# cerbos/cerbos

Measured on AMD Instinct MI355X. Metric: CheckResources decisions/sec at batch=1M; p50 per-decision us, higher is better.
Workload: dtype u32 ids + f64 attributes (CEL int64/uint64/double)

## Files before the change

### __graft_entry__.py

```python
from __future__ import annotations

import glob
import os
import subprocess
import sys

ROOT = os.path.dirname(os.path.abspath(__file__))
if ROOT not in sys.path:
    sys.path.insert(0, ROOT)

CSRC = os.path.join(ROOT, "cerbos_amd", "csrc")
LIB = os.path.join(ROOT, "cerbos_amd", "libcerbos_hip.so")
SOURCES = ["cbh_engine.hip", "cbh_host_env.h", "cbh_host_resident.h", "cbh_host_cross.h", "cbh_host_wire.h", "cbh_host_oneshot.h", "cbh_kernels.h", "cbh_check_wave.h", "cbh_check_flat.h", "cbh_check_walk2.h", "cbh_interp.h", "cbh_vm.h", "cbh_blob.h", "cbh_image.h",
           "cbh_wire.h", "cbh_wire_host.h", "cbh_wire_req.h", "cbh_cross.h"]


def _stale(target, deps):
    if not os.path.exists(target):
        return True
    t = os.path.getmtime(target)
    return any(os.path.getmtime(d) > t for d in deps)


def build() -> None:
    deps = [os.path.join(CSRC, s) for s in SOURCES] + [os.path.join(ROOT, "include", "cerbos_hip.h")]
    if _stale(LIB, deps):
        hipcc = os.environ.get("HIPCC", "/opt/rocm/bin/hipcc")
        cmd = [hipcc, "--offload-arch=gfx950", "-O3", "-std=c++17", "-shared", "-fPIC",
# ... 89 lines not shown
```

### cerbos_amd/csrc/cbh_check_flat.h

```cpp
#pragma once
#include "cbh_check_wave.h"

#define CBH_FLAT_MAX_DEPTH 16
#if defined(CBH_FLAT_WAVES_OVERRIDE)
#define CBH_FLAT_WAVES CBH_FLAT_WAVES_OVERRIDE
#elif !defined(CBH_HOSTSIM)
#define CBH_FLAT_WAVES 4u
#else
#define CBH_FLAT_WAVES 1u
#endif
#define CBH_FLAT_THREADS (CBH_FLAT_WAVES * CBH_BLOCK)

__device__ __forceinline__ u64 wave_or64(u64 v, u32 wave, u32 lane) {
  __shared__ unsigned long long acc[CBH_FLAT_WAVES];
#ifndef CBH_HOSTSIM
  if (lane == 0) __hip_atomic_store(&acc[wave], 0ull, __ATOMIC_RELAXED, __HIP_MEMORY_SCOPE_WORKGROUP);
  (void)wave_ballot(true);
  if (v) (void)__hip_atomic_fetch_or(&acc[wave], (unsigned long long)v, __ATOMIC_RELAXED, __HIP_MEMORY_SCOPE_WORKGROUP);
  (void)wave_ballot(true);
  const u64 r = __hip_atomic_load(&acc[wave], __ATOMIC_RELAXED, __HIP_MEMORY_SCOPE_WORKGROUP);
#else
  if (lane == 0) acc[wave] = 0;
  (void)wave_ballot(true);
  if (v) atomicOr(&acc[wave], (unsigned long long)v);
// ... 1169 lines not shown
__global__ __launch_bounds__(256) void cbh_unpack_results_kernel(PkUnpackArgs a) {
  const u32 i = blockIdx.x * 256u + threadIdx.x;
  if (i >= a.n) return;
  const u32 w = a.policy[i];
  a.effect[i] = (u8)cbh_pk_effect(w); a.status[i] = (u8)cbh_pk_status(w);
  a.policy[i] = cbh_pk_policy(w, a.bits); a.scope[i] = cbh_pk_scope(w, a.bits);
}
struct CompactArgs {
  const CBH_G u32* req_u32; const CBH_G u32* roles; const CBH_G u32* tuple_action; const CBH_G u64* col_val;
  const CBH_G u8* action_class; const CBH_G u8* role_class;
  const CBH_G u8* col_tag; CBH_G u32* ctag;
  CBH_G u32* creq; CBH_G u32* cval; CBH_G u32* info;
  u32 n_requests, n_cached, K, narrow;
  const CBH_G u32* scope_parent; const CBH_G u32* scope_flags; u32 n_scopes;
};
__global__ __launch_bounds__(256) void cbh_compact_scan_kernel(CompactArgs a) {
  const u32 r = blockIdx.x * 256u + threadIdx.x;
  if (r >= a.n_requests) return;
  const size_t NR = a.n_requests;
  u32 m = 0;
  for (u32 k = 0; k < a.n_cached; ++k) m |= (u32)(a.col_val[k * NR + r] >> 32) ? 1u << k : 0u;
#define RQ(f) a.req_u32[(size_t)(f) * NR + r]
  if ((RQ(CBH_RQ_KIND) | RQ(CBH_RQ_R_VERSION) | (RQ(CBH_RQ_R_SCOPE) & ~CBH_SCOPE_EXACT)) >> 16) m |= CBH_CI_MISFIT;
  if (RQ(CBH_RQ_ROLE_CNT) > 4u || RQ(CBH_RQ_ACT_CNT) > 4u) m |= CBH_CI_MISFIT;
  if (RQ(CBH_RQ_ACT_OFF) != 4u * r || RQ(CBH_RQ_ACT_CNT) != 4u) m |= CBH_CI_ACT4;
#undef RQ
#ifdef CBH_HOSTSIM
  a.info[0] |= m;
#else
  if (m & ~__hip_atomic_load(a.info, __ATOMIC_RELAXED, __HIP_MEMORY_SCOPE_AGENT)) atomicOr((unsigned int*)a.info, m);
// ... 11 lines not shown
  u32 ac[4], rc[4];
  for (u32 k = 0; k < 4; ++k) {
    const u32 aid = a.tuple_action[k < act_cnt ? act_off + k : 0u], rid = a.roles[k < role_cnt ? role_off + k : 0u];
    const u32 ca = a.K ? a.action_class[aid < a.K ? aid : kmax] : 31u, cr = a.K ? a.role_class[rid < a.K ? rid : kmax] : 31u;
    ac[k] = (k < act_cnt && aid < a.K && ca < 31u) ? ca : 31u;
    rc[k] = (k < role_cnt && rid < a.K && cr < 31u) ? cr : 31u;
  }
  const u32 si = r_scope & ~CBH_SCOPE_EXACT;
  u32 first = CBH_NONE;
  bool strict = false;
  if (si < a.n_scopes) {
    strict = (r_scope & CBH_SCOPE_EXACT) != 0 && (a.scope_flags[si] & FLAG_RES) != 0;
    first = si;
    while (first != CBH_NONE && !(a.scope_flags[first] & FLAG_RES)) first = a.scope_parent[first];
  }
  CBH_G u32* rec = a.creq + 4u * (size_t)r;
  rec[0] = pid; rec[1] = cbh_creq_w1(kind, r_ver);
  rec[2] = cbh_creq_w2(first, role_cnt, act_cnt, rc[2], rc[3]);
  rec[3] = cbh_creq_w3(first, strict, ac[0], ac[1], ac[2], ac[3], rc[0], rc[1]);
  u32 plane = 0;
  for (u32 k = 0; k < a.n_cached; ++k)
    if ((a.narrow >> k) & 1u) { a.cval[plane * NR + r] = (u32)a.col_val[k * NR + r]; ++plane; }
  for (u32 g = 0; 4u * g < a.n_cached; ++g) {
    u32 w = 0;
    for (u32 j = 0; j < 4u && 4u * g + j < a.n_cached; ++j) w |= (u32)a.col_tag[(4u * g + j) * NR + r] << (8u * j);
    a.ctag[g * NR + r] = w;
  }
}
static inline cbh_check_kernel_fn cbh_flat_compact_variant(cbh_check_kernel_fn fn) {
  return fn == cbh_check_flat_kernel ? cbh_check_flat_kernel_c
// ... 29 lines not shown
  const int m = cbh_flat_cross_mode(fn);
  return m == 0 ? cbh_check_flat_kernel_x : m == 1 ? cbh_check_flat_kernel_staged_x : m == 2 ? cbh_check_flat_kernel_masks_x : m == 3 ? cbh_check_flat_kernel_dr_x : nullptr;
}
static inline const char* cbh_flat_cross_name(cbh_check_kernel_fn fn) {
  const int m = cbh_flat_cross_mode(fn);
  return m == 0 ? "cbh_check_flat_kernel_x" : m == 1 ? "cbh_check_flat_kernel_staged_x" : m == 2 ? "cbh_check_flat_kernel_masks_x" : m == 3 ? "cbh_check_flat_kernel_dr_x" : "";
}
#define CBH_FLAT_STAGE_MIN 32u
static inline bool cbh_flat_use_masks(const void* segs, u32 max_bucket) {
  static const char* e = getenv("CBH_FLAT_MASKS");
  static const bool force_staged = getenv("CBH_FORCE_STAGED") != nullptr;
  if ((e && *e == '0') || force_staged) return false;
  return segs != nullptr && ((e && *e == '1') || max_bucket > CBH_FLAT_STAGE_MIN);
}

static inline size_t cbh_flat_chain_bytes(u32 table_max_depth, u32 table_scopes) {
  return (size_t)(table_max_depth < CBH_FLAT_MAX_DEPTH ? table_max_depth : CBH_FLAT_MAX_DEPTH) * CBH_BLOCK * (table_scopes <= 256u ? 1 : 4);
}
static inline size_t cbh_flat_class_bytes(u32 table_strings) {
  return table_strings <= CBH_FLAT_LDS_STRINGS ? (((size_t)2 * table_strings + 15) & ~(size_t)15) : 0;
}
static inline size_t cbh_flat_mask_bytes(u32 threads) { return (size_t)(threads / CBH_BLOCK) * CBH_SEG_LDS_BYTES; }
static inline bool cbh_is_mask_kernel(cbh_check_kernel_fn fn) {
  return fn == cbh_check_flat_kernel_masks || fn == cbh_check_flat_kernel_any_masks || fn == cbh_check_flat_trail_kernel_masks || fn == cbh_check_flat_trail_kernel_any_masks;
}
static inline cbh_check_kernel_fn cbh_flat_trail_variant(cbh_check_kernel_fn fn) {
  return (fn == cbh_check_flat_kernel || fn == cbh_check_flat_kernel_dr) ? cbh_check_flat_trail_kernel : fn == cbh_check_flat_kernel_any ? cbh_check_flat_trail_kernel_any
       : fn == cbh_check_flat_kernel_staged ? cbh_check_flat_trail_kernel_staged : fn == cbh_check_flat_kernel_any_staged ? cbh_check_flat_trail_kernel_any_staged
       : fn == cbh_check_flat_kernel_masks ? cbh_check_flat_trail_kernel_masks : fn == cbh_check_flat_kernel_any_masks ? cbh_check_flat_trail_kernel_any_masks : fn;
}
static inline bool cbh_is_flat_trail_kernel(cbh_check_kernel_fn fn) {
  return fn == cbh_check_flat_trail_kernel || fn == cbh_check_flat_trail_kernel_any || fn == cbh_check_flat_trail_kernel_staged ||
         fn == cbh_check_flat_trail_kernel_any_staged || fn == cbh_check_flat_trail_kernel_masks || fn == cbh_check_flat_trail_kernel_any_masks;
}
// ... 18 lines not shown
```

### cerbos_amd/csrc/cbh_check_walk2.h

```cpp
#pragma once
#include "cbh_check_flat.h"

#if defined(CBH_HOSTSIM) || defined(CBH_FLAT_WAVES_OVERRIDE)
#define CBH_W2_WAVES CBH_FLAT_WAVES
#else
#define CBH_W2_WAVES 2u
#endif
#define CBH_W2_THREADS (CBH_W2_WAVES * CBH_BLOCK)
#define CBH_W2_LDS_GLOB_STRINGS 1024u
#define CBH_W2_MAX_RP_ROLES 32u

struct __attribute__((aligned(32))) TblRowX { u32 gslots, globs, rm_lo, rm_hi, am_lo, am_hi, p0, p1; };
struct __attribute__((aligned(64))) TblRpx { u32 resource, cnt, cond, gslot, am_lo, am_hi, ag, how; LeafRec leaf; };

struct W2Layout { u32 cc_dw, arena_dw, chain_dw, aux_dw, gacc_dw, edr_dw, wave_dw, cls_bytes; };
#ifndef CBH_HOSTSIM
__host__ __device__
#endif
static inline W2Layout w2_layout(u32 ncc, bool arena, u32 table_max_depth, u32 table_scopes, bool pre, u32 n_gwords, u32 table_strings, u32 table_n_dr, u32 na = CBH_W2_NA, bool packed_tags = false) {
  W2Layout l;
  const u32 depth = table_max_depth < CBH_FLAT_MAX_DEPTH ? table_max_depth : CBH_FLAT_MAX_DEPTH;
  l.cc_dw = CBH_CC_DWORDS(ncc, packed_tags);
  l.arena_dw = (pre && arena) ? CBH_ARENA_ENTRIES * CBH_BLOCK * 9u / 4u : 0u;
  l.chain_dw = pre ? 0u : (table_scopes <= 256u ? depth * (CBH_BLOCK / 4u) : depth * CBH_BLOCK);
// ... 954 lines not shown
  } else
  p.kernel = cbh_pick_kernel(no_flat ? (table_flags & ~(u32)CBH_MF_FLAT) : table_flags, n_derived_roles, has_globs, max_actions, max_roles, plain_tags, eval_flags, max_bucket, &p.threads, &flat, masks);
  p.kind = flat ? 1 : 0;
  if (!flat && !no_walk2 && cbh_walk2_applies(table_flags, eval_flags)) {
    p.walk_wide = max_roles > CBH_W2_NR && !no_walk2_wide;
    p.walk_awide = max_actions > CBH_W2_NA && !no_walk2_wide;
    const bool beyond_base = max_actions > CBH_W2_NA || max_roles > CBH_W2_NR;
    const bool beyond_all = max_actions > CBH_W2_AWIDE_NA || max_roles > CBH_W2_WIDE_NR || (max_actions > CBH_W2_NA && max_roles > CBH_W2_NR);
    if (no_walk2_wide ? beyond_base : beyond_all) p.wide_kernel = p.kernel;
    p.kind = 2; p.kernel = want_ep ? cbh_walk2_trail_kernel : cbh_walk2_kernel; p.threads = CBH_W2_THREADS; p.trail = want_ep;
    p.n_gwords = w2_gwords(gslots_generic, gslots_all, plain_tags);
    p.n_gslots = plain_tags ? gslots_generic : gslots_all;
  }
  return p;
}
static inline size_t cbh_general_lds(u32 table_flags, u32 n_columns, bool packed_tags = false) {
  const u32 ncc = n_columns < CBH_CACHE_COLS ? n_columns : CBH_CACHE_COLS;
  return (size_t)CBH_CC_DWORDS(ncc, packed_tags) * 4 + ((table_flags & CBH_MF_NEEDS_ARENA) ? (size_t)CBH_ARENA_ENTRIES * CBH_BLOCK * 9 : 0);
}
static inline size_t cbh_plan_lds(const CbhPlan& p, u32 table_flags, u32 table_max_depth, u32 table_scopes, u32 table_strings, u32 n_columns, u32 inline_cols, u32 table_n_dr, bool pre, u32 na = CBH_W2_NA, bool packed_tags = false) {
  const u32 ncc = n_columns < CBH_CACHE_COLS ? n_columns : CBH_CACHE_COLS;
  if (p.kind == 2) return w2_lds_bytes(w2_layout(pre ? ncc : inline_cols, (table_flags & CBH_MF_NEEDS_ARENA) != 0, table_max_depth, table_scopes, pre, p.n_gwords, table_strings, table_n_dr, na, packed_tags), pre ? 1u : CBH_W2_WAVES);
  const size_t wave = cbh_general_lds(table_flags, n_columns, packed_tags);
  if (p.kind == 1) return (wave + cbh_flat_chain_bytes(table_max_depth, table_scopes)) * (p.threads / CBH_BLOCK) + cbh_flat_class_bytes(table_strings)
                          + (cbh_is_mask_kernel(p.kernel) ? cbh_flat_mask_bytes(p.threads) : 0)
                          + (cbh_is_flat_trail_kernel(p.kernel) ? cbh_flat_trail_bytes(p.threads, table_max_depth) : 0);
  return wave;
}
```

### cerbos_amd/csrc/cbh_engine.hip

```cpp
#include <hip/hip_runtime.h>
#include <hip/hip_ext.h>
#include <dlfcn.h>
#include <map>
#include <tuple>

#include <algorithm>
#include <atomic>
#include <cassert>
#include <chrono>
#include <cstdio>
#include <cstdlib>
#include <cstring>
#include <ctime>
#include <condition_variable>
#include <memory>
#include <mutex>
#include <new>
#include <string>
#include <thread>
#include <vector>

#include "cbh_kernels.h"
#include "cbh_image.h"
#include "cbh_wire_host.h"

#if !defined(__HIP_DEVICE_COMPILE__)

#include "cbh_host_env.h"

static thread_local std::string g_err;
static int fail(const std::string& m) { g_err = m; return -1; }
#define HIPCHK(x) do { hipError_t _e = (x); if (_e != hipSuccess) return fail(std::string(#x) + ": " + hipGetErrorString(_e)); } while (0)

struct Rccl {
  void* lib = nullptr;
  int (*CommInitAll)(void**, int, const int*) = nullptr;
  int (*CommDestroy)(void*) = nullptr;
// ... 165 lines not shown
  cbh_table* table = nullptr;
  Replica* rep = nullptr;
  BatchDev dev{};
  OutDev out{};
  hipStream_t stream = nullptr;
  KernelArgs* d_args = nullptr;
  KernelArgs last_args;
  bool have_args = false;
  PlanShape shape;
  std::vector<std::pair<void*, size_t>> allocs;
  bool wire = false;
  WireBatch w;
  u32 trail_groups = 0; u32* trail_grp = nullptr;
  bool res_packed = false; bool edr_zero = false;
  bool compact = false;
  u64* allow_bits = nullptr;
  u8* dflag = nullptr;
};

static void replica_destroy(Replica* r) {
  if (!r) return;
  (void)hipSetDevice(r->device);
  for (int i = 1; i < Replica::MAX_RESIDENT_STREAMS; ++i) if (r->rstreams[i]) { (void)hipStreamSynchronize(r->rstreams[i]); (void)hipStreamDestroy(r->rstreams[i]); }
  if (r->stream) { (void)hipStreamSynchronize(r->stream); (void)hipStreamDestroy(r->stream); }
  for (auto& sl : r->ring) for (auto& e : sl.ev) if (e) (void)hipEventDestroy(e);
  for (hipStream_t ws : r->wstreams_all) { (void)hipStreamSynchronize(ws); (void)hipStreamDestroy(ws); }
  for (auto& pb : r->wpinned_idle) (void)hipHostFree(pb.first);
  for (hipStream_t ls : {r->up_stream, r->down_stream}) if (ls) { (void)hipStreamSynchronize(ls); (void)hipStreamDestroy(ls); }
  for (hipEvent_t e : r->wevents_idle) (void)hipEventDestroy(e);
  if (r->image && r->owns_image) (void)hipFree(r->image);
// ... 214 lines not shown
```

### cerbos_amd/csrc/cbh_host_resident.h

```cpp
#pragma once

static bool flat_groups_shape(const cbh_table* t, u32 max_actions, u32 max_roles) {
  return flat_action_groups_on() && !t->reps.empty() && cbh_flat_action_groups(t->reps[0]->dev.n_dr, max_actions, max_roles) != 0;
}
static bool plain_tags_select(const cbh_table* t, u32 max_actions, u32 max_roles) {
  const u32 mf = t->meta[CBH_M_FLAGS];
  return ((mf & CBH_MF_FLAT) && max_roles <= 4 && (max_actions <= 4 || flat_groups_shape(t, max_actions, max_roles))) ||
         ((mf & CBH_MF_WALK2) && t->meta[CBH_M_GSLOTS_ALL] > t->meta[CBH_M_GSLOTS_GENERIC]);
}
static bool has_int_or_container_tag(const uint8_t* p, size_t n) {
  size_t i = 0; uint64_t hit = 0;
  for (; i + 8 <= n; i += 8) {
    uint64_t w; std::memcpy(&w, p + i, 8);
    const uint64_t z = (w & 0xFAFAFAFAFAFAFAFAull) ^ 0x0202020202020202ull;
    hit |= (z - 0x0101010101010101ull) & ~z & 0x8080808080808080ull;
  }
  for (; i < n; ++i) hit |= (uint64_t)((p[i] & 0xFAu) == 0x02u);
  return hit != 0;
}
struct TagRows { size_t first, count; };
template <typename Rows>
static bool sens_tag_hit(const cbh_table* t, const uint8_t* tags, u32 n_columns, size_t n_rows, Rows rows) {
  for (u32 c = 0; c < 32 && c < n_columns; ++c) if ((t->meta[CBH_M_SENS_COLS] >> c) & 1u) {
    const TagRows r = rows(c);
// ... 48 lines not shown
  u32 wlo = 0xFFFFFFFFu, whi = 0;
  if (maxa > CBH_W2_NA || maxr > CBH_W2_NR)
    for (size_t r = 0; r < NR; ++r)
      if (act_cnt[r] > CBH_W2_NA || role_cnt[r] > CBH_W2_NR) { if (wlo == 0xFFFFFFFFu) wlo = (u32)r; whi = (u32)r + 1; }
  if (maxa > CBH_MAX_ACTIONS_PER_REQUEST) return fail("cbh_batch: a request carries more than CBH_MAX_ACTIONS_PER_REQUEST actions");
  if (bad) return fail("cbh_batch: a request's role or action slice lies outside the batch");
  if (in->n_strings && in->str_off[in->n_strings] > in->str_bytes_len) return fail("cbh_batch: string offsets exceed str_bytes_len");
  sh.max_actions = maxa; sh.max_roles = maxr; sh.ascending = !unordered;
  sh.wide_lo = whi ? wlo : 0; sh.wide_hi = whi;
  sh.table = t; sh.tags = plain_tags_select(t, maxa, maxr) ? in->col_tag : nullptr; sh.n_columns = in->n_columns; sh.n_req = NR;
  sh.plain.store(-1, std::memory_order_relaxed);
  return 0;
}

static bool compact_inputs_on() { static const bool on = env_int("CBH_COMPACT_INPUTS", 1) != 0; return on; }
static int batch_compact(cbh_device_batch* b, hipStream_t s) {
  const TableDev& dev = b->rep->dev;
  BatchDev& d = b->dev;
  if (!compact_inputs_on() || !(dev.flags & CBH_MF_FLAT) || b->shape.max_actions > 4 || b->shape.max_roles > 4 || !d.n_requests) return 0;
  CompactArgs ca{};
  ca.req_u32 = d.req_u32; ca.roles = d.roles; ca.tuple_action = d.tuple_action; ca.col_val = d.col_val; ca.col_tag = d.col_tag;
  ca.action_class = dev.action_class; ca.role_class = dev.role_class; ca.K = dev.K;
  ca.scope_parent = dev.scope_parent; ca.scope_flags = dev.scope_flags; ca.n_scopes = dev.n_scopes;
  ca.n_requests = d.n_requests; ca.n_cached = d.n_columns < CBH_CACHE_COLS ? d.n_columns : CBH_CACHE_COLS;
  if (dalloc(b, ca.info, 1) != 0) return -1;
  const dim3 grid((d.n_requests + 255u) / 256u);
  u32 info = 0;
  HIPCHK(hipMemsetAsync(ca.info, 0, 4, s));
  hipLaunchKernelGGL(cbh_compact_scan_kernel, grid, dim3(256), 0, s, ca);
  HIPCHK(hipMemcpyAsync(&info, ca.info, 4, hipMemcpyDeviceToHost, s));
  HIPCHK(hipStreamSynchronize(s));
  if (info & CBH_CI_MISFIT) return 0;
  ca.narrow = ~info & ((1u << ca.n_cached) - 1u) & CBH_CI_NARROW_MASK;
  if (dalloc(b, ca.creq, (size_t)4 * d.n_requests) != 0 || dalloc(b, ca.cval, (size_t)__builtin_popcount(ca.narrow) * d.n_requests) != 0 ||
      dalloc(b, ca.ctag, (size_t)((ca.n_cached + 3u) / 4u) * d.n_requests) != 0) return -1;
  hipLaunchKernelGGL(cbh_compact_pack_kernel, grid, dim3(256), 0, s, ca);
  HIPCHK(hipGetLastError());
  d.creq = ca.creq; d.cval = ca.cval; d.ctag = ca.ctag; d.compact_info = ca.narrow | ((info & CBH_CI_ACT4) ? 0u : CBH_CI_ACT4);
  b->compact = true;
  return 0;
}

static int batch_device_buffers(cbh_device_batch* b, size_t gbits_words) {
  BatchDev& d = b->dev; const Replica* rep = b->rep;
  int rc = dalloc(b, d.gbits, gbits_words);
  d.n_gwords = (rep->dev.flags & CBH_MF_WALK2) ? w2_gwords(rep->dev.gslots_generic, rep->dev.gslots_all, b->shape.plain_tags) : 0;
  d.n_gslots = 0;
  if (d.n_gwords) rc |= dalloc(b, d.gres, (size_t)d.n_gwords * d.n_requests); else d.gres = nullptr;
  rc |= dalloc(b, b->out.effect, d.n_tuples);
  rc |= dalloc(b, b->out.policy, d.n_tuples);
  rc |= dalloc(b, b->out.scope, d.n_tuples);
  rc |= dalloc(b, b->out.status, d.n_tuples);
  rc |= dalloc(b, b->out.edr, d.n_requests);
  rc |= dalloc(b, b->d_args, 1);
// ... 98 lines not shown
  static std::mutex mu;
  static std::map<std::tuple<const void*, u32, size_t>, int> memo;
  auto blocks = [&](size_t lds) {
    const auto key = std::make_tuple((const void*)fn, threads, lds);
    std::lock_guard<std::mutex> g(mu);
    auto it = memo.find(key);
    if (it != memo.end()) return it->second;
    int n = 0;
    if (hipOccupancyMaxActiveBlocksPerMultiprocessor(&n, (const void*)fn, (int)threads, lds) != hipSuccess) { (void)hipGetLastError(); n = 0; }
    memo.emplace(key, n);
    return n;
  };
  return blocks(lds_packed) > blocks(lds_wide);
}
static void launch_plan(const CbhPlan& pl, const TableDev& dev, KernelArgs ka, const KernelArgs* d_args, u32 lo, u32 hi, u32 wide_lo, u32 wide_hi,
                        size_t pad, hipStream_t s, hipEvent_t ev0 = nullptr, hipEvent_t ev1 = nullptr, u8* dflag = nullptr) {
  if (hi <= lo) return;
  ka.b.req_lo = lo; ka.b.req_hi = hi;
  ka.flags &= ~(u32)(CBH_FI_MASK & ~(CBH_FI_PACKED_RES | CBH_FI_COMPACT));
  const u32 n = hi - lo;
  auto go = [&](cbh_check_kernel_fn fn, u32 grid, u32 threads, auto lds_of, const KernelArgs& a0, bool last) {
    const size_t wide = lds_of(false), packed = lds_of(true);
    const bool use_packed = cbh_is_flat_compact_kernel(fn) || packed_tags_pay(fn, threads, wide, packed);
    const size_t lds = use_packed ? packed : wide;
    KernelArgs a = a0;
    if (use_packed) a.flags |= CBH_FI_PACKED_TAGS;
    if (ev0 || (ev1 && last)) { hipExtLaunchKernelGGL(fn, dim3(grid), dim3(threads), lds, s, ev0, last ? ev1 : nullptr, 0, a, d_args); ev0 = nullptr; }
    else hipLaunchKernelGGL(fn, dim3(grid), dim3(threads), lds, s, a, d_args);
  };
  auto plan_lds = [&](bool pre, u32 na, size_t extra) {
    return [=, &pl, &dev, &ka](bool packed) { return cbh_plan_lds(pl, dev.flags, dev.max_depth, dev.n_scopes, dev.K, ka.b.n_columns, dev.inline_cols, dev.n_dr, pre, na, packed) + extra; };
// ... 45 lines not shown
    for (u32 g = 0; g < pl.groups; ++g) {
      ag.group = g;
      const bool last = g + 1 == pl.groups && !ag.dflag;
      if (ev0 || (ev1 && last)) { hipExtLaunchKernelGGL(gfn, grid, block, use_packed ? packed : wide, s, ev0, last ? ev1 : nullptr, 0, a, d_args, ag); ev0 = nullptr; }
      else hipLaunchKernelGGL(gfn, grid, block, use_packed ? packed : wide, s, a, d_args, ag);
    }
    if (ag.dflag) {
      FlatGroupStatusArgs sa{};
      sa.req_u32 = ka.b.req_u32; sa.dflag = ag.dflag; sa.n_requests = ka.b.n_requests; sa.lo = lo; sa.hi = hi;
      if (ka.flags & CBH_FI_PACKED_RES) sa.packed = ka.o.policy; else sa.status = ka.o.status;
      if (ev1) hipExtLaunchKernelGGL(cbh_flat_group_status_kernel, dim3((n + 255u) / 256u), dim3(256), 0, s, nullptr, ev1, 0, sa);
      else hipLaunchKernelGGL(cbh_flat_group_status_kernel, dim3((n + 255u) / 256u), dim3(256), 0, s, sa);
    }
    return;
  }
  go((ka.flags & CBH_FI_COMPACT) ? cbh_flat_compact_variant(pl.kernel) : pl.kernel, (n + pl.threads - 1) / pl.threads, pl.threads, plan_lds(false, CBH_W2_NA, pad), ka, true);
}
static size_t lds_pad() { static const size_t pad = (size_t)env_long("CBH_LDS_PAD", 0); return pad; }
static u32 nfa_maxw(const TableDev& d) { return std::max(std::max(d.nfa_words[0], d.nfa_words[1]), d.nfa_words[2]); }
static size_t check_lds_bytes(const BatchDev& d, u32 table_flags) {
  const u32 ncc = d.n_columns < CBH_CACHE_COLS ? d.n_columns : CBH_CACHE_COLS;
  return (size_t)CBH_CC_DWORDS(ncc, false) * 4 + ((table_flags & CBH_MF_NEEDS_ARENA) ? (size_t)CBH_ARENA_ENTRIES * CBH_BLOCK * 9 : 0);
}

static bool pk_fits(const TableDev& dev) {
  static const bool on = env_int("CBH_PACKED_RESULTS", 1) != 0;
  return on && cbh_pk_bits(dev.n_scopes) <= CBH_PK_MAX_BITS;
}

static bool launch_is_compact(const cbh_device_batch* b, const CbhPlan& pl, u32 eval_flags) {
#ifdef CBH_PROFILE_CYCLES
  eval_flags &= ~(u32)CBH_F_DEBUG_CYCLES;
#endif
  return b->compact && pl.kind == 1 && pl.groups <= 1 && !(eval_flags & CBH_F_DEBUG_CYCLES) && cbh_flat_compact_variant(pl.kernel) != nullptr;
}

extern "C" int cbh_check_resident(cbh_table* t, cbh_device_batch* b, const cbh_params* p) {
  if (!t || !b || !p) return fail("null argument");
  if (b->table != t) return fail("batch was uploaded for a different table");
  Replica* rep = b->rep;
  std::lock_guard<std::mutex> lk(rep->mu);
  HIPCHK(hipSetDevice(rep->device));
  hipStream_t s = b->stream;
  b->w.total_known = false;
  if (pre_split_on() && !b->dev.site_cnt && b->dev.n_requests && (rep->dev.flags & CBH_MF_WALK2) && rep->dev.gslots_all &&
      !(rep->dev.flags & CBH_MF_USES_RUNTIME_EDR) && b->dev.gres) {
    u32* cnt = nullptr; u64* list = nullptr;
    if (dalloc(b, cnt, (size_t)rep->dev.gslots_all) != 0 || dalloc(b, list, (size_t)rep->dev.gslots_all * b->dev.n_requests) != 0) return -1;
    b->dev.site_cnt = cnt; b->dev.site_list = list; b->dev.site_cap = b->dev.n_requests;
// ... 18 lines not shown
    if (!b->have_args || std::memcmp(&ka, &b->last_args, sizeof(ka)) != 0) {
      b->last_args = ka; b->have_args = true;
      HIPCHK(hipMemcpyAsync(b->d_args, &b->last_args, sizeof(ka), hipMemcpyHostToDevice, s));
    }
  }
  const u32 maxw = nfa_maxw(rep->dev);
  sl.resolved = d.n_strings && maxw;
  if (sl.resolved) {
    const u32 grid = (d.n_strings + CBH_BLOCK - 1) / CBH_BLOCK;
    const size_t lds = (size_t)(2 + 512) * maxw * sizeof(u64);
    if (timed) hipExtLaunchKernelGGL(cbh_resolve_globs_kernel, dim3(grid), dim3(CBH_BLOCK), lds, s, sl.ev[0], sl.ev[1], 0, rep->dev, d);
    else hipLaunchKernelGGL(cbh_resolve_globs_kernel, dim3(grid), dim3(CBH_BLOCK), lds, s, rep->dev, d);
  }
  sl.pending = false;
  if (d.n_requests) {
    launch_plan(pl, rep->dev, b->last_args, (const KernelArgs*)b->d_args, 0, d.n_requests, b->shape.wide_lo, b->shape.wide_hi, lds_pad(), s, timed ? sl.ev[2] : nullptr, timed ? sl.ev[3] : nullptr, b->dflag);
    sl.pending = timed;
  }
  HIPCHK(hipGetLastError());
  return 0;
}

extern "C" int cbh_check_resident_many(cbh_table* t, cbh_device_batch* const* bs, uint32_t n, const cbh_params* p) {
  if (!t || (!bs && n) || !p) return fail("null argument");
  for (uint32_t i = 0; i < n; ++i) if (cbh_check_resident(t, bs[i], p) != 0) return -1;
  return 0;
}

extern "C" int cbh_table_set_resident_streams(cbh_table* t, uint32_t n) {
  if (!t) return fail("null argument");
  if (n < 1 || n > (uint32_t)Replica::MAX_RESIDENT_STREAMS) return fail("resident streams: 1 .. " + std::to_string(Replica::MAX_RESIDENT_STREAMS));
// ... 5 lines not shown
extern "C" const char* cbh_plan_describe(cbh_table* t, cbh_device_batch* b, const cbh_params* p) {
  static thread_local std::string s;
  if (!t || !b || !p) return "";
  const CbhPlan pl = plan_for(b->rep->dev, b->shape, p->flags & ~(u32)CBH_FI_MASK);
  const Replica* rep = b->rep;
  const bool pre_split = pre_split_on() && b->dev.n_requests && (rep->dev.flags & CBH_MF_WALK2) && rep->dev.gslots_all && !(rep->dev.flags & CBH_MF_USES_RUNTIME_EDR) && b->dev.gres;
  if (pl.kind == 2) s = std::string(pl.wide_kernel ? "cbh_check_kernel*(wide requests)+" : "") + (pl.walk_wide ? (pl.trail ? "cbh_walk2_wide_trail_kernel(5-8 roles)+" : "cbh_walk2_wide_kernel(5-8 roles)+") : "") + (pl.walk_awide ? (pl.trail ? "cbh_walk2_awide_trail_kernel(9-16 actions)+" : "cbh_walk2_awide_kernel(9-16 actions)+") : "") + (pl.n_gwords && b->dev.gres ? (pre_split ? "cbh_walk2_collect_kernel+cbh_walk2_interp_kernel+" : "cbh_walk2_pre_kernel+") : "") + (pl.trail ? "cbh_walk2_trail_kernel" : "cbh_walk2_kernel");
  else if (pl.kind == 1 && cbh_is_flat_trail_kernel(pl.kernel)) s = cbh_is_mask_kernel(pl.kernel) ? "cbh_check_flat_trail_kernel*_masks" : "cbh_check_flat_trail_kernel*";
  else if (pl.kind == 0 && pl.kernel == cbh_check_trail_kernel) s = "cbh_check_trail_kernel";
  else if (pl.kind == 1) s = pl.kernel == cbh_check_flat_kernel ? "cbh_check_flat_kernel" : pl.kernel == cbh_check_flat_kernel_dr ? "cbh_check_flat_kernel_dr" : pl.kernel == cbh_check_flat_kernel_any ? "cbh_check_flat_kernel_any"
                           : pl.kernel == cbh_check_flat_kernel_staged ? "cbh_check_flat_kernel_staged" : pl.kernel == cbh_check_flat_kernel_masks ? "cbh_check_flat_kernel_masks"
                           : pl.kernel == cbh_check_flat_kernel_any_masks ? "cbh_check_flat_kernel_any_masks" : "cbh_check_flat_kernel_any_staged";
  else s = "cbh_check_kernel*";
  if (pl.kind == 1 && pl.groups > 1) { char m[32]; snprintf(m, sizeof m, ", %u action groups", pl.groups); s += m; }
  if (launch_is_compact(b, pl, p->flags)) { char m[64]; snprintf(m, sizeof m, "[compact inputs, narrow columns 0x%x]", b->dev.compact_info & CBH_CI_NARROW_MASK); s += m; }
  return s.c_str();
}

extern "C" int cbh_synchronize(cbh_table* t) {
  if (!t) return fail("null argument");
  for (Replica* rep : t->reps) {
    std::lock_guard<std::mutex> lk(rep->mu);
    HIPCHK(hipSetDevice(rep->device));
    for (int i = 0; i < Replica::MAX_RESIDENT_STREAMS; ++i) if (rep->rstreams[i]) HIPCHK(hipStreamSynchronize(rep->rstreams[i]));
    { std::vector<hipStream_t> ws; { std::lock_guard<std::mutex> lw(rep->wstream_mu); ws = rep->wstreams_all; } for (hipStream_t x : ws) HIPCHK(hipStreamSynchronize(x)); }
    collect_times(rep);
  }
  return 0;
}

// ... 127 lines not shown
```

Measured before the change: 188.0 billion.

## Add batch-uniform bucket route kernel precomputing rule masks for flat check

The compact scan now records whether all requests share one resource kind, version and scope, plus the maximum role count, in a second info word. When the batch is uniform and the table has depth at most one with no derived roles, a one-block route kernel resolves the rule bucket once and writes per-class action and role bitmasks. A new flat kernel variant then evaluates rows from that shared header and LDS masks instead of doing a per-request directory lookup and per-row matching. This adds an extra scan pass, an atomic, a tiny launch and a host readback, and it only applies when the batch is homogeneous.

```diff
diff --git a/__graft_entry__.py b/__graft_entry__.py
--- a/__graft_entry__.py
+++ b/__graft_entry__.py
@@ -11,7 +11,7 @@
 
 CSRC = os.path.join(ROOT, "cerbos_amd", "csrc")
 LIB = os.path.join(ROOT, "cerbos_amd", "libcerbos_hip.so")
-SOURCES = ["cbh_engine.hip", "cbh_host_env.h", "cbh_host_resident.h", "cbh_host_cross.h", "cbh_host_wire.h", "cbh_host_oneshot.h", "cbh_kernels.h", "cbh_check_wave.h", "cbh_check_flat.h", "cbh_check_walk2.h", "cbh_interp.h", "cbh_vm.h", "cbh_blob.h", "cbh_image.h",
+SOURCES = ["cbh_engine.hip", "cbh_host_env.h", "cbh_host_resident.h", "cbh_host_cross.h", "cbh_host_wire.h", "cbh_host_oneshot.h", "cbh_kernels.h", "cbh_check_wave.h", "cbh_check_flat.h", "cbh_check_bucket.h", "cbh_check_walk2.h", "cbh_interp.h", "cbh_vm.h", "cbh_blob.h", "cbh_image.h",
            "cbh_wire.h", "cbh_wire_host.h", "cbh_wire_req.h", "cbh_cross.h"]
 
 
diff --git a/cerbos_amd/csrc/cbh_check_bucket.h b/cerbos_amd/csrc/cbh_check_bucket.h
--- /dev/null
+++ b/cerbos_amd/csrc/cbh_check_bucket.h
@@ -0,0 +1,223 @@
+#pragma once
+#include "cbh_check_walk2.h"
+
+#define CBH_BUCKET_MAX_RECORDS 32u
+#define CBH_BUCKET_MASK_BYTES 256u
+struct __attribute__((aligned(32))) FlatRouteHdr {
+  u32 valid;
+  u32 row_begin, n_records;
+  u32 sp;
+  u32 max_roles;
+  u32 allow_m, deny_m;
+  u32 pad;
+};
+struct FlatRoute { FlatRouteHdr h; u32 am[32]; u32 rm[32]; };
+#define CBH_ROUTE_DWORDS (sizeof(FlatRoute) / 4)
+struct FlatRouteArg { const CBH_G u32* rec; };
+
+__host__ __device__ __forceinline__ size_t cbh_bucket_lds_bytes(u32 table_flags, u32 n_columns, u32 table_max_depth, u32 table_scopes, u32 table_strings) {
+  return (cbh_general_lds(table_flags, n_columns, true) + cbh_flat_chain_bytes(table_max_depth, table_scopes)) * CBH_FLAT_WAVES +
+         cbh_flat_class_bytes(table_strings) + CBH_BUCKET_MASK_BYTES;
+}
+
+struct FlatRouteArgs { TableDev t; const CBH_G u32* creq; const CBH_G u32* info; CBH_G u32* route; u32 n_requests, pad; };
+__global__ __launch_bounds__(CBH_BLOCK) void cbh_flat_route_kernel(FlatRouteArgs a) {
+  __shared__ u32 hdr[8];
+  const TableDev& t = a.t;
+  const u32 tid = threadIdx.x;
+  if (tid == 0) {
+    const u32 i2 = a.info[1];
+    const u32 w1 = a.creq[1], scope = a.creq[2] & 0xFFFFu;
+    uint4 bucket; bucket.x = bucket.y = bucket.z = bucket.w = 0;
+    bool ok = a.n_requests != 0 && !(i2 & CBH_CI2_MIXED) && t.max_depth <= 1u && t.n_dr == 0u && scope < t.n_scopes;
+    ok = ok && dir_find(t, CBH_B_RESOURCE, w1 >> 16, w1 & 0xFFFFu, scope, bucket);
+    ok = ok && bucket.y <= CBH_BUCKET_MAX_RECORDS && (u64)bucket.x + bucket.y <= (u64)t.n_rows;
+    u32 allow_m = 0, deny_m = 0;
+    for (u32 j = 0; ok && j < bucket.y; ++j) {
+      const CBH_G u32* rw = t.rows + (size_t)(bucket.x + j) * 16u;
+      const u32 fl = rw[0];
+      if ((fl & (CBH_ROW_F_ROLE_BY_CLASS | CBH_ROW_F_ACTION_BY_CLASS)) != (CBH_ROW_F_ROLE_BY_CLASS | CBH_ROW_F_ACTION_BY_CLASS) || rw[2] != CBH_NONE) ok = false;
+      if ((fl & 3u) == CBH_EFFECT_ALLOW) allow_m |= 1u << j; else if ((fl & 3u) == CBH_EFFECT_DENY) deny_m |= 1u << j;
+    }
+    u32 max_roles = 0;
+    for (u32 r = 1; r <= 4u; ++r) if ((i2 >> r) & 1u) max_roles = r;
+    hdr[0] = ok ? 1u : 0u; hdr[1] = ok ? bucket.x : 0u; hdr[2] = ok ? bucket.y : 0u;
+    hdr[3] = ok ? (t.scope_flags[scope] >> 2) & 3u : 0u; hdr[4] = max_roles; hdr[5] = ok ? allow_m : 0u; hdr[6] = ok ? deny_m : 0u; hdr[7] = 0u;
+  }
+  __syncthreads();
+  const u32 cls = tid & 31u, word = tid < 32u ? 6u : 4u;
+  u32 m = 0;
+  for (u32 j = 0; j < hdr[2]; ++j) m |= ((t.rows[(size_t)(hdr[1] + j) * 16u + word] >> cls) & 1u) << j;
+  a.route[8u + tid] = m;
+  if (tid < 8u) a.route[tid] = hdr[tid];
+}
+
+__device__ __forceinline__ void flat_bucket_body(const KernelArgs& ka_regs, Ctx& c, const CBH_G u32* route) {
+  const TableDev& t = ka_regs.t;
+  const BatchDev& b = ka_regs.b;
+  const OutDev& o = ka_regs.o;
+  const u32 flags = ka_regs.flags;
+  const u32 wave = threadIdx.x / CBH_BLOCK;
+  const u32 rix = b.req_lo + blockIdx.x * CBH_FLAT_THREADS + threadIdx.x;
+  const bool valid = rix < b.req_hi;
+  const u32 req = valid ? rix : b.req_lo;
+  const u32 NR = b.n_requests;
+  const u32 w0r = b.req_lo + blockIdx.x * CBH_FLAT_THREADS + wave * CBH_BLOCK;
+  const u32 w0 = w0r < b.req_hi ? w0r : b.req_lo;
+  const u32 wd = valid ? c.tid : 0u;
+  const u32x4u rec = load_u32x4(b.creq + 4u * (size_t)req);
+  cc_fill_compact(c, b, NR, w0, wd);
+  const u32 mword = route[8u + (threadIdx.x & 63u)];
+  const FlatRouteHdr rh = uload_rec<FlatRouteHdr>(route, 0);
+  CBH_L u32* bm = (CBH_L u32*)(cbh_dyn_lds + ((u32)cbh_bucket_lds_bytes(t.flags, b.n_columns, t.max_depth, t.n_scopes, t.K) - CBH_BUCKET_MASK_BYTES));
+  const u32 pid = rec.x;
+  const u32 w2 = valid ? rec.z : ((rec.z & 0xFFFFu) | 0xFFC00000u), w3 = valid ? rec.w : (rec.w | 0x3FFFFFFFu);
+  const u32 first = cbh_creq_first(w2, w3, (flags & CBH_F_LENIENT_SCOPE_SEARCH) != 0);
+  const u32 role_cnt = (w2 >> 16) & 7u, act_cnt = (w2 >> 19) & 7u;
+  u32 ac[4], rc[4];
+#pragma unroll
+  for (u32 k = 0; k < 4; ++k) ac[k] = (w3 >> (5u * k)) & 31u;
+  rc[0] = (w3 >> 20) & 31u; rc[1] = (w3 >> 25) & 31u; rc[2] = (w2 >> 22) & 31u; rc[3] = w2 >> 27;
+  u32 act_off = 4u * req;
+  if (threadIdx.x < 64u) bm[threadIdx.x] = mword;
+  __syncthreads();
+  const u32 all = (1u << act_cnt) - 1u;
+  u32 lane_ac = 0, lane_rc = 0;
+  u32 walks = 0;
+#pragma unroll
+  for (u32 k = 0; k < 4; ++k) {
+    if (k < act_cnt) lane_ac |= 1u << ac[k];
+    if (k < role_cnt) { lane_rc |= 1u << rc[k]; walks |= all << (4 * k); }
+  }
+  const u64 wave_cls = wave_or64((u64)lane_ac | ((u64)lane_rc << 32), wave, c.tid);
+  const u32 wave_ac = (u32)wave_cls, wave_rc = (u32)(wave_cls >> 32);
+  const bool part = first != CBH_NONE;
+  const bool go = wave_ballot(part && walks != 0) != 0;
+
+  u32 sat = 0, errm = 0, unsm = 0;
+  if (go && rh.n_records) {
+    const u32 last = rh.row_begin + rh.n_records - 1u;
+    TblRowFull nxt = uload_rec<TblRowFull>(t.rows, rh.row_begin);
+    for (u32 j = 0; j < rh.n_records; ++j) {
+      const TblRowFull rf = nxt;
+      const u32 row = rh.row_begin + j;
+      nxt = uload_rec<TblRowFull>(t.rows, row < last ? row + 1u : last);
+      const TblRow& rw = rf.hot;
+      if ((rw.rm_lo & wave_rc) == 0 || (rw.am_lo & wave_ac) == 0) continue;
+      const u32 bit = 1u << j;
+      if (rw.cond == CBH_NONE) { sat |= bit; continue; }
+      u32 lv = 4u;
+      if (rw.flags & CBH_ROW_F_LEAF_EMBEDDED) lv = flat_leaf<false, true>(c, rf.leaf, req, pid);
+      else if (rw.flags & CBH_ROW_F_TREE_EMBEDDED) lv = flat_tree<false, true>(c, rf.leaf, req, pid);
+      sat |= (lv & 1u) ? bit : 0u; errm |= (lv & 2u) ? bit : 0u; unsm |= (lv == 4u) ? bit : 0u;
+    }
+  }
+
+  u32 has_allow = 0, allow = 0, deny = 0, err = 0, unsup = 0;
+  if (go) {
+    u32 amk[4];
+#pragma unroll
+    for (u32 k = 0; k < 4; ++k) amk[k] = bm[ac[k]];
+    const bool anybad = wave_ballot(part && (errm | unsm) != 0) != 0;
+#pragma unroll
+    for (u32 r = 0; r < 4; ++r) {
+      if (r >= rh.max_roles) break;
+      const u32 rmk = part ? bm[32u + rc[r]] : 0u;
+#pragma unroll
+      for (u32 k = 0; k < 4; ++k) {
+        const u32 bit = 1u << (4u * r + k);
+        const u32 cand = (walks & bit) ? (rmk & amk[k]) : 0u;
+        const u32 hits = cand & sat;
+        const u32 dh = hits & rh.deny_m;
+        const u32 below = dh ? (((dh & (0u - dh)) << 1) - 1u) : ~0u;
+        has_allow |= (hits & rh.allow_m & below) ? bit : 0u;
+        deny |= dh ? bit : 0u;
+        if (anybad) { err |= (cand & errm & below) ? bit : 0u; unsup |= (cand & unsm & below) ? bit : 0u; }
+      }
+    }
+    const u32 ha = has_allow & walks & ~deny;
+    if (rh.sp == SP_OVERRIDE_PARENT) allow |= ha;
+  }
+
+  const bool decided = !part;
+  const u32 pol_none = (u32)(decided ? CBH_P_NO_MATCH : (role_cnt ? CBH_P_RESOURCE : CBH_P_EMPTY)) << 28 | ((!decided && role_cnt) ? first : 0u);
+  const u32 pol_hit = ((u32)CBH_P_RESOURCE << 28) | first;
+  const u32 st_ok = (t.flags & CBH_MF_TRACE_ALL) ? CBH_ST_WANTS_TRACE : CBH_ST_OK;
+  bool alw[4], won[4];
+  u32 sc1[4];
+#pragma unroll
+  for (u32 k = 0; k < 4; ++k) {
+    const u32 ak = allow & (0x1111u << k), dk = deny & (0x1111u << k);
+    const u32 sel = ak ? ak : dk;
+    alw[k] = ak != 0; won[k] = sel != 0;
+    sc1[k] = (won[k] && k < act_cnt) ? first + 1u : 0u;
+  }
+  u32 st4 = st_ok * 0x01010101u;
+  if (wave_ballot((err | unsup) != 0) != 0) {
+    st4 = 0;
+#pragma unroll
+    for (u32 k = 0; k < 4; ++k) {
+      const u32 ak = (allow >> k) & 0x1111u;
+      const u32 seen = ak ? (((ak & (0u - ak)) << 1) - 1u) : 0xFFFFu;
+      const u32 ek = (err >> k) & 0x1111u & seen, uk = (unsup >> k) & 0x1111u & seen;
+      st4 |= (u32)(uk ? CBH_ST_UNSUPPORTED : (ek ? CBH_ST_CEL_ERROR : st_ok)) << (8 * k);
+    }
+  }
+  const u64 edr = 0;
+
+  if (!(b.compact_info & CBH_CI_ACT4)) act_off = b.req_u32[(size_t)CBH_RQ_ACT_OFF * NR + req];
+  const bool packed = valid && act_cnt == 4 && (act_off & 3u) == 0;
+#ifndef CBH_HOSTSIM
+  typedef u32 u32x4 __attribute__((ext_vector_type(4)));
+#else
+  struct u32x4 { u32 x, y, z, w; };
+#endif
+  if (flags & CBH_FI_PACKED_RES) {
+    const u32 sh = 7u + cbh_pk_bits(t.n_scopes);
+    const u32 pk_hit = ((pol_hit >> 28) << 4) | ((pol_hit & 0x0FFFFFFFu) << 7), pk_none = ((pol_none >> 28) << 4) | ((pol_none & 0x0FFFFFFFu) << 7);
+    u32 pw[4];
+#pragma unroll
+    for (u32 k = 0; k < 4; ++k)
+      pw[k] = (u32)(alw[k] ? CBH_EFFECT_ALLOW : CBH_EFFECT_DENY) | (((st4 >> (8 * k)) & 0xFFu) << 2) | (won[k] ? pk_hit : pk_none) | (sc1[k] << sh);
+    if (packed) {
+      if (o.edr) store_nt(o.edr + req, edr);
+      u32x4 v; v.x = pw[0]; v.y = pw[1]; v.z = pw[2]; v.w = pw[3];
+      store_nt((CBH_G u32x4*)(o.policy + act_off), v);
+    } else if (valid) {
+      if (o.edr) o.edr[req] = edr;
+#pragma unroll
+      for (u32 k = 0; k < 4; ++k) if (k < act_cnt) o.policy[act_off + k] = pw[k];
+    }
+  } else {
+    u32 eff4 = 0, pol[4], scp[4];
+#pragma unroll
+    for (u32 k = 0; k < 4; ++k) {
+      eff4 |= (u32)(alw[k] ? CBH_EFFECT_ALLOW : CBH_EFFECT_DENY) << (8 * k);
+      pol[k] = won[k] ? pol_hit : pol_none;
+      scp[k] = sc1[k] - 1u;
+    }
+    if (packed) {
+      if (o.edr) store_nt(o.edr + req, edr);
+      store_nt((CBH_G u32*)(o.effect + act_off), eff4);
+      if (o.status) store_nt((CBH_G u32*)(o.status + act_off), st4);
+      if (o.policy) { u32x4 v; v.x = pol[0]; v.y = pol[1]; v.z = pol[2]; v.w = pol[3]; store_nt((CBH_G u32x4*)(o.policy + act_off), v); }
+      if (o.scope) { u32x4 v; v.x = scp[0]; v.y = scp[1]; v.z = scp[2]; v.w = scp[3]; store_nt((CBH_G u32x4*)(o.scope + act_off), v); }
+    } else if (valid) {
+      if (o.edr) o.edr[req] = edr;
+#pragma unroll
+      for (u32 k = 0; k < 4; ++k) {
+        if (k < act_cnt) {
+          o.effect[act_off + k] = (u8)((eff4 >> (8 * k)) & 0xFFu);
+          if (o.status) o.status[act_off + k] = (u8)((st4 >> (8 * k)) & 0xFFu);
+          if (o.policy) o.policy[act_off + k] = pol[k];
+          if (o.scope) o.scope[act_off + k] = scp[k];
+        }
+      }
+    }
+  }
+}
+
+__global__ CBH_FLAT_ATTRS(8) void cbh_check_flat_kernel_b(const KernelArgs a, const KernelArgs* __restrict__ ka, const FlatRouteArg r) {
+  CBH_FLAT_CTX_C(a, ka);
+  flat_bucket_body(a, c, r.rec);
+}
diff --git a/cerbos_amd/csrc/cbh_check_flat.h b/cerbos_amd/csrc/cbh_check_flat.h
--- a/cerbos_amd/csrc/cbh_check_flat.h
+++ b/cerbos_amd/csrc/cbh_check_flat.h
@@ -1207,6 +1207,7 @@
   u32 n_requests, n_cached, K, narrow;
   const CBH_G u32* scope_parent; const CBH_G u32* scope_flags; u32 n_scopes;
 };
+#define CBH_CI2_MIXED 0x100u
 __global__ __launch_bounds__(256) void cbh_compact_scan_kernel(CompactArgs a) {
   const u32 r = blockIdx.x * 256u + threadIdx.x;
   if (r >= a.n_requests) return;
@@ -1248,6 +1249,19 @@
     first = si;
     while (first != CBH_NONE && !(a.scope_flags[first] & FLAG_RES)) first = a.scope_parent[first];
   }
+  {
+    const u32 si0 = a.req_u32[(size_t)CBH_RQ_R_SCOPE * NR] & ~CBH_SCOPE_EXACT;
+    u32 first0 = CBH_NONE;
+    if (si0 < a.n_scopes) { first0 = si0; while (first0 != CBH_NONE && !(a.scope_flags[first0] & FLAG_RES)) first0 = a.scope_parent[first0]; }
+    u32 m2 = 1u << role_cnt;
+    if (first != CBH_NONE && (cbh_creq_w1(kind, r_ver) != cbh_creq_w1(a.req_u32[(size_t)CBH_RQ_KIND * NR], a.req_u32[(size_t)CBH_RQ_R_VERSION * NR]) ||
+                              (first & 0xFFFFu) != (first0 != CBH_NONE ? first0 & 0xFFFFu : 0u))) m2 |= CBH_CI2_MIXED;
+#ifdef CBH_HOSTSIM
+    a.info[1] |= m2;
+#else
+    if (m2 & ~__hip_atomic_load(a.info + 1, __ATOMIC_RELAXED, __HIP_MEMORY_SCOPE_AGENT)) atomicOr((unsigned int*)a.info + 1, m2);
+#endif
+  }
   CBH_G u32* rec = a.creq + 4u * (size_t)r;
   rec[0] = pid; rec[1] = cbh_creq_w1(kind, r_ver);
   rec[2] = cbh_creq_w2(first, role_cnt, act_cnt, rc[2], rc[3]);
@@ -1307,10 +1321,10 @@
   return segs != nullptr && ((e && *e == '1') || max_bucket > CBH_FLAT_STAGE_MIN);
 }
 
-static inline size_t cbh_flat_chain_bytes(u32 table_max_depth, u32 table_scopes) {
+__host__ __device__ static inline size_t cbh_flat_chain_bytes(u32 table_max_depth, u32 table_scopes) {
   return (size_t)(table_max_depth < CBH_FLAT_MAX_DEPTH ? table_max_depth : CBH_FLAT_MAX_DEPTH) * CBH_BLOCK * (table_scopes <= 256u ? 1 : 4);
 }
-static inline size_t cbh_flat_class_bytes(u32 table_strings) {
+__host__ __device__ static inline size_t cbh_flat_class_bytes(u32 table_strings) {
   return table_strings <= CBH_FLAT_LDS_STRINGS ? (((size_t)2 * table_strings + 15) & ~(size_t)15) : 0;
 }
 static inline size_t cbh_flat_mask_bytes(u32 threads) { return (size_t)(threads / CBH_BLOCK) * CBH_SEG_LDS_BYTES; }
diff --git a/cerbos_amd/csrc/cbh_check_walk2.h b/cerbos_amd/csrc/cbh_check_walk2.h
--- a/cerbos_amd/csrc/cbh_check_walk2.h
+++ b/cerbos_amd/csrc/cbh_check_walk2.h
@@ -992,7 +992,7 @@
   }
   return p;
 }
-static inline size_t cbh_general_lds(u32 table_flags, u32 n_columns, bool packed_tags = false) {
+__host__ __device__ static inline size_t cbh_general_lds(u32 table_flags, u32 n_columns, bool packed_tags = false) {
   const u32 ncc = n_columns < CBH_CACHE_COLS ? n_columns : CBH_CACHE_COLS;
   return (size_t)CBH_CC_DWORDS(ncc, packed_tags) * 4 + ((table_flags & CBH_MF_NEEDS_ARENA) ? (size_t)CBH_ARENA_ENTRIES * CBH_BLOCK * 9 : 0);
 }
diff --git a/cerbos_amd/csrc/cbh_engine.hip b/cerbos_amd/csrc/cbh_engine.hip
--- a/cerbos_amd/csrc/cbh_engine.hip
+++ b/cerbos_amd/csrc/cbh_engine.hip
@@ -21,6 +21,7 @@
 #include <vector>
 
 #include "cbh_kernels.h"
+#include "cbh_check_bucket.h"
 #include "cbh_image.h"
 #include "cbh_wire_host.h"
 
@@ -216,6 +217,7 @@
   u32 trail_groups = 0; u32* trail_grp = nullptr;
   bool res_packed = false; bool edr_zero = false;
   bool compact = false;
+  u32* route = nullptr; u32 route_valid = 0;
   u64* allow_bits = nullptr;
   u8* dflag = nullptr;
 };
diff --git a/cerbos_amd/csrc/cbh_host_resident.h b/cerbos_amd/csrc/cbh_host_resident.h
--- a/cerbos_amd/csrc/cbh_host_resident.h
+++ b/cerbos_amd/csrc/cbh_host_resident.h
@@ -86,6 +86,7 @@
 }
 
 static bool compact_inputs_on() { static const bool on = env_int("CBH_COMPACT_INPUTS", 1) != 0; return on; }
+static bool flat_bucket_on() { static const bool on = env_int("CBH_FLAT_BUCKET", 1) != 0; return on; }
 static int batch_compact(cbh_device_batch* b, hipStream_t s) {
   const TableDev& dev = b->rep->dev;
   BatchDev& d = b->dev;
@@ -95,10 +96,10 @@
   ca.action_class = dev.action_class; ca.role_class = dev.role_class; ca.K = dev.K;
   ca.scope_parent = dev.scope_parent; ca.scope_flags = dev.scope_flags; ca.n_scopes = dev.n_scopes;
   ca.n_requests = d.n_requests; ca.n_cached = d.n_columns < CBH_CACHE_COLS ? d.n_columns : CBH_CACHE_COLS;
-  if (dalloc(b, ca.info, 1) != 0) return -1;
+  if (dalloc(b, ca.info, 2) != 0) return -1;
   const dim3 grid((d.n_requests + 255u) / 256u);
   u32 info = 0;
-  HIPCHK(hipMemsetAsync(ca.info, 0, 4, s));
+  HIPCHK(hipMemsetAsync(ca.info, 0, 8, s));
   hipLaunchKernelGGL(cbh_compact_scan_kernel, grid, dim3(256), 0, s, ca);
   HIPCHK(hipMemcpyAsync(&info, ca.info, 4, hipMemcpyDeviceToHost, s));
   HIPCHK(hipStreamSynchronize(s));
@@ -110,6 +111,14 @@
   HIPCHK(hipGetLastError());
   d.creq = ca.creq; d.cval = ca.cval; d.ctag = ca.ctag; d.compact_info = ca.narrow | ((info & CBH_CI_ACT4) ? 0u : CBH_CI_ACT4);
   b->compact = true;
+  if (flat_bucket_on() && dev.max_depth <= 1u && dev.n_dr == 0u) {
+    if (dalloc(b, b->route, CBH_ROUTE_DWORDS) != 0) return -1;
+    FlatRouteArgs ra{};
+    ra.t = dev; ra.creq = ca.creq; ra.info = ca.info; ra.route = b->route; ra.n_requests = d.n_requests;
+    hipLaunchKernelGGL(cbh_flat_route_kernel, dim3(1), dim3(CBH_BLOCK), 0, s, ra);
+    HIPCHK(hipGetLastError());
+    HIPCHK(hipMemcpyAsync(&b->route_valid, b->route, 4, hipMemcpyDeviceToHost, s));
+  }
   return 0;
 }
 
@@ -238,7 +247,7 @@
   return blocks(lds_packed) > blocks(lds_wide);
 }
 static void launch_plan(const CbhPlan& pl, const TableDev& dev, KernelArgs ka, const KernelArgs* d_args, u32 lo, u32 hi, u32 wide_lo, u32 wide_hi,
-                        size_t pad, hipStream_t s, hipEvent_t ev0 = nullptr, hipEvent_t ev1 = nullptr, u8* dflag = nullptr) {
+                        size_t pad, hipStream_t s, hipEvent_t ev0 = nullptr, hipEvent_t ev1 = nullptr, u8* dflag = nullptr, const u32* route = nullptr) {
   if (hi <= lo) return;
   ka.b.req_lo = lo; ka.b.req_hi = hi;
   ka.flags &= ~(u32)(CBH_FI_MASK & ~(CBH_FI_PACKED_RES | CBH_FI_COMPACT));
@@ -314,6 +323,16 @@
     }
     return;
   }
+  if (route && (ka.flags & CBH_FI_COMPACT)) {
+    KernelArgs a = ka;
+    a.flags |= CBH_FI_PACKED_TAGS;
+    const size_t lds = cbh_bucket_lds_bytes(dev.flags, ka.b.n_columns, dev.max_depth, dev.n_scopes, dev.K) + pad;
+    const dim3 grid((n + pl.threads - 1) / pl.threads), block(pl.threads);
+    FlatRouteArg ra{route};
+    if (ev0 || ev1) hipExtLaunchKernelGGL(cbh_check_flat_kernel_b, grid, block, lds, s, ev0, ev1, 0, a, d_args, ra);
+    else hipLaunchKernelGGL(cbh_check_flat_kernel_b, grid, block, lds, s, a, d_args, ra);
+    return;
+  }
   go((ka.flags & CBH_FI_COMPACT) ? cbh_flat_compact_variant(pl.kernel) : pl.kernel, (n + pl.threads - 1) / pl.threads, pl.threads, plan_lds(false, CBH_W2_NA, pad), ka, true);
 }
 static size_t lds_pad() { static const size_t pad = (size_t)env_long("CBH_LDS_PAD", 0); return pad; }
@@ -333,6 +352,12 @@
   eval_flags &= ~(u32)CBH_F_DEBUG_CYCLES;
 #endif
   return b->compact && pl.kind == 1 && pl.groups <= 1 && !(eval_flags & CBH_F_DEBUG_CYCLES) && cbh_flat_compact_variant(pl.kernel) != nullptr;
+}
+
+static bool launch_is_bucket(const cbh_device_batch* b, const CbhPlan& pl, u32 eval_flags) {
+  const TableDev& dev = b->rep->dev;
+  return launch_is_compact(b, pl, eval_flags) && !(eval_flags & CBH_F_DEBUG_CYCLES) && pl.kernel == cbh_check_flat_kernel && dev.max_depth <= 1u && dev.n_dr == 0u &&
+         b->route != nullptr && b->route_valid == 1u;
 }
 
 extern "C" int cbh_check_resident(cbh_table* t, cbh_device_batch* b, const cbh_params* p) {
@@ -381,7 +406,8 @@
   }
   sl.pending = false;
   if (d.n_requests) {
-    launch_plan(pl, rep->dev, b->last_args, (const KernelArgs*)b->d_args, 0, d.n_requests, b->shape.wide_lo, b->shape.wide_hi, lds_pad(), s, timed ? sl.ev[2] : nullptr, timed ? sl.ev[3] : nullptr, b->dflag);
+    launch_plan(pl, rep->dev, b->last_args, (const KernelArgs*)b->d_args, 0, d.n_requests, b->shape.wide_lo, b->shape.wide_hi, lds_pad(), s, timed ? sl.ev[2] : nullptr, timed ? sl.ev[3] : nullptr, b->dflag,
+                launch_is_bucket(b, pl, p->flags) ? b->route : nullptr);
     sl.pending = timed;
   }
   HIPCHK(hipGetLastError());
@@ -417,6 +443,7 @@
   else s = "cbh_check_kernel*";
   if (pl.kind == 1 && pl.groups > 1) { char m[32]; snprintf(m, sizeof m, ", %u action groups", pl.groups); s += m; }
   if (launch_is_compact(b, pl, p->flags)) { char m[64]; snprintf(m, sizeof m, "[compact inputs, narrow columns 0x%x]", b->dev.compact_info & CBH_CI_NARROW_MASK); s += m; }
+  if (launch_is_bucket(b, pl, p->flags)) s += " [bucket masks]";
   return s.c_str();
 }
 
```

New measurement: 175.2 billion. -6.8%, worse.
